# lucidrains/audiolm-pytorch

Measured on NVIDIA H100. Metric: CoarseTransformer tokens/sec fwd+bwd seq2048, higher is better.
Workload: dtype bf16

## Files before the change

audiolm_pytorch_b200/csrc/attn_fwd_wgmma.cu:

```cuda
#include "alm_common.cuh"
#include "ptx_sm90.cuh"

namespace alm {

constexpr int ATT_BM = 128;
constexpr int ATT_BN = 128;
constexpr int ATT_THREADS = 384;
template <int D>
struct AttFwdCfg {
  static constexpr int KV_STAGES = D == 128 ? 3 : 4;
  static constexpr int HALF_BYTES = 128 * SwizzledTile<D>::ROW_BYTES;
  static constexpr int TILE_BYTES = 128 * D * 2;
  static constexpr int SMEM_BYTES = TILE_BYTES * (1 + 2 * KV_STAGES) + 256;
};

struct AttnFwdParams {
  __nv_bfloat16* o;
  float* lse;
  const uint32_t* kmask;
  int kb_stride;
  const float* bias;
  long long bias_hs, bias_rs;
  long long ldo, lse_stride;
  int b, h, n_q, n_k;
  int causal;
  float scale_log2;
  int n_q_pad;
  uint32_t drop_row0;
  DropoutArgs drop;
};

__device__ __forceinline__ float att_ex2(float x) {
  float y;
  asm("ex2.approx.ftz.f32 %0, %1;" : "=f"(y) : "f"(x));
  return y;
}

__device__ __forceinline__ uint64_t attn_fwd_keep_bits(const DropoutArgs& d, uint32_t qrow, uint32_t kbase, int c_lane) {
  const uint32_t odd = qrow & 1u;
  uint64_t bits = 0;
#pragma unroll
  for (int kk = 0; kk < ATT_BN / 16; ++kk) {
    const uint32_t j0 = kbase + 16 * kk + c_lane;
    const uint4 own = dropout_draw(d, qrow, j0 + odd);
    const uint32_t ra = __shfl_xor_sync(0xffffffffu, odd ? own.x : own.y, 4);
    const uint32_t rb = __shfl_xor_sync(0xffffffffu, odd ? own.z : own.w, 4);
    const uint4 other = odd ? make_uint4(0u, ra, 0u, rb) : make_uint4(ra, 0u, rb, 0u);
#pragma unroll
    for (int c = 0; c < 2; ++c) {
      const uint4 dr = (uint32_t)c == odd ? own : other;
#pragma unroll
      for (int half = 0; half < 2; ++half)
#pragma unroll
        for (int h = 0; h < 2; ++h)
          if (dropout_pick(d, dr, qrow + 8 * h, j0 + 8 * half + c)) bits |= 1ull << (8 * kk + 4 * half + 2 * h + c);
    }
  }
  return bits;
}

template <int ATT_D, bool HAS_BIAS, bool DROPOUT>
__global__ void __launch_bounds__(ATT_THREADS, 1)
mqa_attn_fwd_kernel(const __grid_constant__ CUtensorMap tmQ, const __grid_constant__ CUtensorMap tmK,
                    const __grid_constant__ CUtensorMap tmV, const AttnFwdParams p) {
  using Tile = SwizzledTile<ATT_D>;
  using Cfg = AttFwdCfg<ATT_D>;
  constexpr int ATT_KV_STAGES = Cfg::KV_STAGES, ATT_TILE_BYTES = Cfg::TILE_BYTES, HALF = Cfg::HALF_BYTES;
  constexpr bool REG_HANDOFF = ATT_D == 128;
  extern __shared__ __align__(1024) uint8_t smem_raw[];
  uint8_t* smem = smem_raw;
  if ((smem_u32(smem) & 1023u) != 0) __trap();
  uint8_t* sQ = smem;
  uint8_t* sK = sQ + ATT_TILE_BYTES;
  uint8_t* sV = sK + ATT_KV_STAGES * ATT_TILE_BYTES;
  uint64_t* bars = reinterpret_cast<uint64_t*>(sV + ATT_KV_STAGES * ATT_TILE_BYTES);
  uint64_t* q_full = bars;
  uint64_t* kv_full = bars + 1;
  uint64_t* kv_empty = kv_full + ATT_KV_STAGES;

  const int warp = threadIdx.x >> 5;
  const int lane = threadIdx.x & 31;
  const int wg = warp >> 2;
  const int n_qblocks = (p.n_q + ATT_BM - 1) / ATT_BM;
  const int qb = n_qblocks - 1 - (int)blockIdx.x;
  const int head = blockIdx.y;
  const int batch = blockIdx.z;
  const int q0 = qb * ATT_BM;
  const int off = p.n_k - p.n_q;
  int kv_end = p.n_k;
  if (p.causal) kv_end = min(p.n_k, q0 + ATT_BM + off);
  const int n_tiles = kv_end > 0 ? (kv_end + ATT_BN - 1) / ATT_BN : 0;

  if (threadIdx.x == 0) {
    tma_prefetch_desc(&tmQ);
    tma_prefetch_desc(&tmK);
    tma_prefetch_desc(&tmV);
    mbar_init(q_full, 1);
    for (int i = 0; i < ATT_KV_STAGES; ++i) {
      mbar_init(&kv_full[i], 1);
      mbar_init(&kv_empty[i], 8);
    }
    fence_mbar_init();
  }
  __syncthreads();

  if (wg == 0) {
    if constexpr (REG_HANDOFF) setmaxnreg_dec<40>();
    if (warp == 0 && n_tiles > 0) {
      if (elect_one_sync()) {
        mbar_arrive_expect_tx(q_full, ATT_TILE_BYTES);
#pragma unroll
        for (int hf = 0; hf < Tile::HALVES; ++hf)
          tma_load_3d(sQ + hf * HALF, &tmQ, q_full, head * ATT_D + hf * Tile::HW, q0, batch);
      }
      __syncwarp();
      int stage = 0;
      uint32_t phase = 0;
      for (int j = 0; j < n_tiles; ++j) {
        mbar_wait(&kv_empty[stage], phase ^ 1u);
        if (elect_one_sync()) {
          mbar_arrive_expect_tx(&kv_full[stage], 2 * ATT_TILE_BYTES);
#pragma unroll
          for (int hf = 0; hf < Tile::HALVES; ++hf) {
            tma_load_3d(sK + stage * ATT_TILE_BYTES + hf * HALF, &tmK, &kv_full[stage], hf * Tile::HW, j * ATT_BN, batch);
            tma_load_3d(sV + stage * ATT_TILE_BYTES + hf * HALF, &tmV, &kv_full[stage], hf * Tile::HW, j * ATT_BN, batch);
          }
        }
        __syncwarp();
        if (++stage == ATT_KV_STAGES) { stage = 0; phase ^= 1u; }
      }
    }
    return;
  }

  if constexpr (REG_HANDOFF) setmaxnreg_inc<232>();
  const int cw = wg - 1;
  const int r_base = cw * 64 + (warp & 3) * 16 + (lane >> 2);
  const int c_lane = 2 * (lane & 3);
  constexpr float kLog2e = 1.4426950408889634f;
  float m_run[2] = {-INFINITY, -INFINITY}, l_run[2] = {0.f, 0.f};
  float o_acc[ATT_D / 2];
#pragma unroll
  for (int d = 0; d < ATT_D / 2; ++d) o_acc[d] = 0.f;
  int q_limit[2];
  [[maybe_unused]] const float* brow[2];
#pragma unroll
  for (int h = 0; h < 2; ++h) {
    const int qi = q0 + r_base + 8 * h;
    q_limit[h] = min(p.causal ? qi + off : p.n_k - 1, p.n_k - 1);
    if constexpr (HAS_BIAS) brow[h] = p.bias + (long long)head * p.bias_hs + (long long)min(qi, p.n_q - 1) * p.bias_rs;
  }
  const uint32_t* mrow = p.kmask ? p.kmask + (long long)batch * p.kb_stride : nullptr;
  const uint32_t q_addr = smem_u32(sQ) + cw * 64 * Tile::ROW_BYTES;
  [[maybe_unused]] const uint32_t drop_row =
      p.drop_row0 + ((uint32_t)batch * p.h + head) * (uint32_t)p.n_q_pad + q0 + r_base;

  if (n_tiles > 0) mbar_wait(q_full, 0);
  int stage = 0;
  uint32_t phase = 0;
  for (int j = 0; j < n_tiles; ++j) {
    mbar_wait(&kv_full[stage], phase);
    const uint32_t k_addr = smem_u32(sK + stage * ATT_TILE_BYTES);
    const uint32_t v_addr = smem_u32(sV + stage * ATT_TILE_BYTES);
    float s[ATT_BN / 2];
    wgmma_fence();
#pragma unroll
    for (int k = 0; k < ATT_D / 16; ++k)
      wgmma_ss<ATT_BN>(s, Tile::kmajor(q_addr, k, HALF), Tile::kmajor(k_addr, k, HALF), k > 0 ? 1u : 0u);
    wgmma_commit();
    [[maybe_unused]] uint64_t keep = 0;
    if constexpr (DROPOUT) keep = attn_fwd_keep_bits(p.drop, drop_row, j * ATT_BN, c_lane);
    wgmma_wait<0>();
    wgmma_fence_acc(s);

    const int kbase = j * ATT_BN;
    const bool tile_full = mrow == nullptr && kbase + ATT_BN <= p.n_k && (!p.causal || kbase + ATT_BN - 1 <= q0 + off);
    uint32_t valid[4] = {0xFFFFFFFFu, 0xFFFFFFFFu, 0xFFFFFFFFu, 0xFFFFFFFFu};
    if (!tile_full && mrow != nullptr) {
      const uint4 mv = __ldg(reinterpret_cast<const uint4*>(mrow + j * 4));
      valid[0] = mv.x; valid[1] = mv.y; valid[2] = mv.z; valid[3] = mv.w;
    }
    uint32_t pa[ATT_BN / 16][4];
#pragma unroll
    for (int h = 0; h < 2; ++h) {
#pragma unroll
      for (int g = 0; g < ATT_BN / 8; ++g)
#pragma unroll
        for (int c = 0; c < 2; ++c) {
          const int col = 8 * g + c_lane + c;
          float v = s[4 * g + 2 * h + c] * p.scale_log2;
          if constexpr (HAS_BIAS) {
            if (kbase + col < p.bias_rs) v = fmaf(__ldg(brow[h] + kbase + col), kLog2e, v);
          }
          if (!tile_full) {
            const bool ok = kbase + col <= q_limit[h] && ((valid[col >> 5] >> (col & 31)) & 1u);
            if (!ok) v = -INFINITY;
          }
          s[4 * g + 2 * h + c] = v;
        }
      float m_tile = -INFINITY;
#pragma unroll
      for (int g = 0; g < ATT_BN / 8; ++g) m_tile = fmaxf(m_tile, fmaxf(s[4 * g + 2 * h], s[4 * g + 2 * h + 1]));
      m_tile = fmaxf(m_tile, __shfl_xor_sync(0xffffffffu, m_tile, 1));
      m_tile = fmaxf(m_tile, __shfl_xor_sync(0xffffffffu, m_tile, 2));
      const float m_new = fmaxf(m_run[h], m_tile);
      const float m_use = (m_new == -INFINITY) ? 0.f : m_new;
      const float alpha = att_ex2(m_run[h] - m_use);
      float l_tile = 0.f;
#pragma unroll
      for (int g = 0; g < ATT_BN / 8; ++g)
#pragma unroll
        for (int c = 0; c < 2; ++c) {
          const float pv = att_ex2(s[4 * g + 2 * h + c] - m_use);
          s[4 * g + 2 * h + c] = pv;
          l_tile += pv;
        }
      l_run[h] = fmaf(l_run[h], alpha, l_tile);
      m_run[h] = m_new;
#pragma unroll
      for (int g = 0; g < ATT_D / 8; ++g) {
        o_acc[4 * g + 2 * h] *= alpha;
        o_acc[4 * g + 2 * h + 1] *= alpha;
      }
    }
    if constexpr (DROPOUT) {
#pragma unroll
      for (int e = 0; e < ATT_BN / 2; ++e) s[e] = ((keep >> e) & 1u) ? s[e] * p.drop.scale : 0.f;
    }
#pragma unroll
    for (int kk = 0; kk < ATT_BN / 16; ++kk) {
      pa[kk][0] = pack_bf16x2(s[8 * kk + 0], s[8 * kk + 1]);
      pa[kk][1] = pack_bf16x2(s[8 * kk + 2], s[8 * kk + 3]);
      pa[kk][2] = pack_bf16x2(s[8 * kk + 4], s[8 * kk + 5]);
      pa[kk][3] = pack_bf16x2(s[8 * kk + 6], s[8 * kk + 7]);
    }
    wgmma_fence_acc(o_acc);
    wgmma_fence();
#pragma unroll
    for (int kk = 0; kk < ATT_BN / 16; ++kk)
      wgmma_rs<ATT_D, 1>(o_acc, pa[kk], Tile::mnmajor(v_addr, kk, HALF), 1u);
    wgmma_commit();
    wgmma_wait<0>();
    wgmma_fence_acc(o_acc);
    if (lane == 0) mbar_arrive(&kv_empty[stage]);
    if (++stage == ATT_KV_STAGES) { stage = 0; phase ^= 1u; }
  }

#pragma unroll
  for (int h = 0; h < 2; ++h) {
    float l_tot = l_run[h];
    l_tot += __shfl_xor_sync(0xffffffffu, l_tot, 1);
    l_tot += __shfl_xor_sync(0xffffffffu, l_tot, 2);
    const int qi = q0 + r_base + 8 * h;
    if (qi < p.n_q) {
      const float inv = l_tot > 0.f ? 1.f / l_tot : 0.f;
      __nv_bfloat16* dst = p.o + ((long long)batch * p.n_q + qi) * p.ldo + head * ATT_D + c_lane;
#pragma unroll
      for (int g = 0; g < ATT_D / 8; ++g)
        *reinterpret_cast<uint32_t*>(dst + 8 * g) = pack_bf16x2(o_acc[4 * g + 2 * h] * inv, o_acc[4 * g + 2 * h + 1] * inv);
      if (p.lse != nullptr && (lane & 3) == 0) {
        const float lse = l_tot > 0.f ? (m_run[h] + log2f(l_tot)) : INFINITY;
        p.lse[((long long)batch * p.h + head) * p.lse_stride + qi] = lse;
      }
    }
  }
}

}

namespace alm {
__global__ void pack_key_mask_kernel(const uint8_t* __restrict__ mask, uint32_t* __restrict__ bits, int n_k, int words,
                                     long long total) {
  const long long i = (long long)blockIdx.x * (blockDim.x >> 5) + (threadIdx.x >> 5);
  if (i >= total) return;
  const long long b = i / words;
  const int k = (int)(i - b * words) * 32 + (threadIdx.x & 31);
  const bool on = k < n_k && mask[b * n_k + k] != 0;
  const uint32_t v = __ballot_sync(0xffffffffu, on);
  if ((threadIdx.x & 31) == 0) bits[i] = v;
}
}

extern "C" int alm_pack_key_mask(const void* key_mask, void* bits, int b, int n_k, alm_stream_t stream_) {
  using namespace alm;
  cudaStream_t stream = reinterpret_cast<cudaStream_t>(stream_);
  ALM_REQUIRE(key_mask && bits && b > 0 && n_k > 0, ALM_ERR_ARG);
  const int words = (n_k + 127) / 128 * 4;
  const long long total = (long long)b * words;
  const long long blocks = ceil_div(total, 8LL);
  ALM_REQUIRE(blocks <= INT_MAX, ALM_ERR_UNSUPPORTED);
  pack_key_mask_kernel<<<(unsigned)blocks, 256, 0, stream>>>(reinterpret_cast<const uint8_t*>(key_mask),
                                                            reinterpret_cast<uint32_t*>(bits), n_k, words, total);
  ALM_CHECK_LAUNCH();
  ALM_LAUNCHED(1);
  return ALM_OK;
}

namespace alm {
template <int D>
static int attn_fwd_launch(const void* q, int64_t ldq, const void* k, int64_t ldk, int64_t k_bstride, const void* v,
                           int64_t ldv, int64_t v_bstride, const void* key_mask, void* o, int64_t ldo, float* lse,
                           const float* bias, int b, bool drop, AttnFwdParams p, cudaStream_t stream) {
  using Tile = SwizzledTile<D>;
  constexpr int SMEM = AttFwdCfg<D>::SMEM_BYTES;
  const int h = p.h, n_q = p.n_q, n_k = p.n_k;
  static bool attr_set = false;
  if (!attr_set) {
    ALM_CUDA_OK(cudaFuncSetAttribute(mqa_attn_fwd_kernel<D, false, false>, cudaFuncAttributeMaxDynamicSharedMemorySize, SMEM));
    ALM_CUDA_OK(cudaFuncSetAttribute(mqa_attn_fwd_kernel<D, true, false>, cudaFuncAttributeMaxDynamicSharedMemorySize, SMEM));
    ALM_CUDA_OK(cudaFuncSetAttribute(mqa_attn_fwd_kernel<D, false, true>, cudaFuncAttributeMaxDynamicSharedMemorySize, SMEM));
    ALM_CUDA_OK(cudaFuncSetAttribute(mqa_attn_fwd_kernel<D, true, true>, cudaFuncAttributeMaxDynamicSharedMemorySize, SMEM));
    attr_set = true;
  }
  constexpr int kMaxGridZ = 65535;
  const int n_launch = ceil_div(b, kMaxGridZ);
  for (int b0 = 0; b0 < b; b0 += kMaxGridZ) {
    const int nb = min(b - b0, kMaxGridZ);
    CUtensorMap tmQ, tmK, tmV;
    {
      uint64_t dims[3] = {(uint64_t)h * D, (uint64_t)n_q, (uint64_t)nb};
      uint64_t strides[3] = {2, (uint64_t)ldq * 2, (uint64_t)n_q * ldq * 2};
      uint32_t box[3] = {Tile::HW, ATT_BM, 1};
      int rc = make_tensor_map(&tmQ, reinterpret_cast<const __nv_bfloat16*>(q) + (long long)b0 * n_q * ldq, 2, 3, dims,
                               strides, box, Tile::SWIZZLE);
      if (rc != ALM_OK) return rc;
    }
    {
      uint64_t dims[3] = {(uint64_t)D, (uint64_t)n_k, (uint64_t)nb};
      uint64_t strides[3] = {2, (uint64_t)ldk * 2, (uint64_t)k_bstride * 2};
      uint32_t box[3] = {Tile::HW, ATT_BN, 1};
      int rc = make_tensor_map(&tmK, reinterpret_cast<const __nv_bfloat16*>(k) + (long long)b0 * k_bstride, 2, 3, dims,
                               strides, box, Tile::SWIZZLE);
      if (rc != ALM_OK) return rc;
      strides[1] = (uint64_t)ldv * 2;
      strides[2] = (uint64_t)v_bstride * 2;
      rc = make_tensor_map(&tmV, reinterpret_cast<const __nv_bfloat16*>(v) + (long long)b0 * v_bstride, 2, 3, dims,
                           strides, box, Tile::SWIZZLE);
      if (rc != ALM_OK) return rc;
    }
    p.o = reinterpret_cast<__nv_bfloat16*>(o) + (long long)b0 * n_q * ldo;
    p.lse = lse != nullptr ? lse + (long long)b0 * h * p.lse_stride : nullptr;
    p.kmask = key_mask != nullptr ? reinterpret_cast<const uint32_t*>(key_mask) + (long long)b0 * p.kb_stride : nullptr;
    p.b = nb;
    p.drop_row0 = (uint32_t)((long long)b0 * h * p.n_q_pad);
    const dim3 grid((n_q + ATT_BM - 1) / ATT_BM, h, nb);
    if (bias != nullptr && drop)
      mqa_attn_fwd_kernel<D, true, true><<<grid, ATT_THREADS, SMEM, stream>>>(tmQ, tmK, tmV, p);
    else if (bias != nullptr)
      mqa_attn_fwd_kernel<D, true, false><<<grid, ATT_THREADS, SMEM, stream>>>(tmQ, tmK, tmV, p);
    else if (drop)
      mqa_attn_fwd_kernel<D, false, true><<<grid, ATT_THREADS, SMEM, stream>>>(tmQ, tmK, tmV, p);
    else
      mqa_attn_fwd_kernel<D, false, false><<<grid, ATT_THREADS, SMEM, stream>>>(tmQ, tmK, tmV, p);
    ALM_CHECK_LAUNCH();
  }
  ALM_LAUNCHED(n_launch);
  return ALM_OK;
}
}

extern "C" int alm_mqa_attn_fwd_dh(const void* q, int64_t ldq, const void* k, int64_t ldk, int64_t k_bstride,
                                   const void* v, int64_t ldv, int64_t v_bstride, const void* key_mask, void* o,
                                   int64_t ldo, float* lse, int64_t lse_stride, const float* bias,
                                   int64_t bias_hstride, int64_t bias_rstride, int b, int h, int n_q, int n_k,
                                   int causal, float scale, float dropout_p, uint64_t seed, uint32_t site,
                                   int dim_head, alm_stream_t stream_) {
  using namespace alm;
  cudaStream_t stream = reinterpret_cast<cudaStream_t>(stream_);
  ALM_REQUIRE(dim_head == 32 || dim_head == 64 || dim_head == 128, ALM_ERR_UNSUPPORTED);
  ALM_REQUIRE(q && k && v && o, ALM_ERR_ARG);
  ALM_REQUIRE(b > 0 && h > 0 && n_q > 0 && n_k > 0 && n_k >= n_q, ALM_ERR_ARG);
  ALM_REQUIRE(dropout_p >= 0.f && dropout_p < 1.f, ALM_ERR_ARG);
  ALM_REQUIRE((long long)b * h * ((n_q + 127) / 128 * 128) < (1ll << 32), ALM_ERR_UNSUPPORTED);
  ALM_REQUIRE(ldq % 8 == 0 && ldk % 8 == 0 && ldv % 8 == 0 && ldo % 8 == 0, ALM_ERR_ALIGN);
  ALM_REQUIRE(k_bstride % 8 == 0 && v_bstride % 8 == 0, ALM_ERR_ALIGN);
  ALM_REQUIRE((reinterpret_cast<uintptr_t>(o) & 15u) == 0, ALM_ERR_ALIGN);
  if (bias != nullptr) {
    ALM_REQUIRE(bias_rstride >= n_k && bias_rstride % 4 == 0 && bias_hstride % 4 == 0, ALM_ERR_ALIGN);
    ALM_REQUIRE((reinterpret_cast<uintptr_t>(bias) & 15u) == 0, ALM_ERR_ALIGN);
  }

  AttnFwdParams p;
  p.kb_stride = (n_k + 127) / 128 * 4;
  p.bias = bias;
  p.bias_hs = bias_hstride;
  p.bias_rs = bias_rstride;
  p.ldo = ldo;
  p.lse_stride = lse_stride;
  p.h = h; p.n_q = n_q; p.n_k = n_k;
  p.causal = causal;
  p.scale_log2 = scale * 1.4426950408889634f;
  p.n_q_pad = (n_q + 127) / 128 * 128;
  p.drop = make_dropout_args(dropout_p, seed, site);
  const bool drop = dropout_p > 0.f;
#define ALM_ATT_FWD(DD) \
  attn_fwd_launch<DD>(q, ldq, k, ldk, k_bstride, v, ldv, v_bstride, key_mask, o, ldo, lse, bias, b, drop, p, stream)
  if (dim_head == 32) return ALM_ATT_FWD(32);
  if (dim_head == 64) return ALM_ATT_FWD(64);
  return ALM_ATT_FWD(128);
#undef ALM_ATT_FWD
}

extern "C" int alm_mqa_attn_fwd(const void* q, int64_t ldq, const void* k, int64_t ldk, int64_t k_bstride,
                                const void* v, int64_t ldv, int64_t v_bstride, const void* key_mask, void* o,
                                int64_t ldo, float* lse, int64_t lse_stride, const float* bias, int64_t bias_hstride,
                                int64_t bias_rstride, int b, int h, int n_q, int n_k, int causal, float scale,
                                float dropout_p, uint64_t seed, uint32_t site, alm_stream_t stream_) {
  return alm_mqa_attn_fwd_dh(q, ldq, k, ldk, k_bstride, v, ldv, v_bstride, key_mask, o, ldo, lse, lse_stride, bias,
                             bias_hstride, bias_rstride, b, h, n_q, n_k, causal, scale, dropout_p, seed, site, 64,
                             stream_);
}
```

audiolm_pytorch_b200/csrc/ptx_sm90.cuh:

```cuda
#pragma once
#include <cuda.h>
#include <cuda_runtime.h>
#include <cuda_bf16.h>
#include <stdint.h>
#include <stdio.h>

namespace alm {

__device__ __forceinline__ uint32_t smem_u32(const void* p) {
  return static_cast<uint32_t>(__cvta_generic_to_shared(p));
}
__device__ __forceinline__ uint32_t lane_id() { return threadIdx.x & 31u; }

__device__ __forceinline__ uint64_t global_timer_ns() {
  uint64_t t;
  asm volatile("mov.u64 %0, %%globaltimer;" : "=l"(t));
  return t;
}

__device__ __forceinline__ void mbar_init(uint64_t* bar, uint32_t arrive_count) {
  asm volatile("mbarrier.init.shared::cta.b64 [%0], %1;" ::"r"(smem_u32(bar)), "r"(arrive_count) : "memory");
}
__device__ __forceinline__ void fence_mbar_init() {
  asm volatile("fence.mbarrier_init.release.cluster;" ::: "memory");
}
__device__ __forceinline__ void mbar_arrive(uint64_t* bar) {
  asm volatile("mbarrier.arrive.shared::cta.b64 _, [%0];" ::"r"(smem_u32(bar)) : "memory");
}
__device__ __forceinline__ void mbar_arrive_expect_tx(uint64_t* bar, uint32_t tx_bytes) {
  asm volatile("mbarrier.arrive.expect_tx.shared::cta.b64 _, [%0], %1;" ::"r"(smem_u32(bar)), "r"(tx_bytes)
               : "memory");
}
__device__ __forceinline__ bool mbar_try_wait(uint64_t* bar, uint32_t parity) {
  uint32_t done;
  asm volatile(
      "{\n\t"
      ".reg .pred p;\n\t"
      "mbarrier.try_wait.parity.shared::cta.b64 p, [%1], %2;\n\t"
      "selp.u32 %0, 1, 0, p;\n\t"
      "}\n"
      : "=r"(done)
      : "r"(smem_u32(bar)), "r"(parity)
      : "memory");
  return done != 0;
}
#ifndef ALM_MBAR_TIMEOUT_NS
#define ALM_MBAR_TIMEOUT_NS 4000000000ull
#endif
__device__ __forceinline__ void mbar_wait(uint64_t* bar, uint32_t parity) {
  if (mbar_try_wait(bar, parity)) return;
  uint64_t t0 = 0;
  uint32_t spins = 0;
  while (!mbar_try_wait(bar, parity)) {
    if ((++spins & 0x3FFu) == 0) {
      uint64_t now = global_timer_ns();
      if (t0 == 0) t0 = now;
      else if (now - t0 > ALM_MBAR_TIMEOUT_NS) __trap();
    }
  }
}

__device__ __forceinline__ void fence_proxy_async_smem() {
  asm volatile("fence.proxy.async.shared::cta;" ::: "memory");
}

__device__ __forceinline__ void tma_prefetch_desc(const CUtensorMap* m) {
  asm volatile("prefetch.tensormap [%0];" ::"l"(reinterpret_cast<uint64_t>(m)) : "memory");
}
__device__ __forceinline__ void tma_load_2d(void* smem_dst, const CUtensorMap* m, uint64_t* bar, int32_t c0,
                                            int32_t c1) {
  asm volatile(
      "cp.async.bulk.tensor.2d.shared::cluster.global.mbarrier::complete_tx::bytes [%0], [%1, {%3, %4}], [%2];"
      ::"r"(smem_u32(smem_dst)), "l"(reinterpret_cast<uint64_t>(m)), "r"(smem_u32(bar)), "r"(c0), "r"(c1)
      : "memory");
}
__device__ __forceinline__ void tma_load_3d(void* smem_dst, const CUtensorMap* m, uint64_t* bar, int32_t c0,
                                            int32_t c1, int32_t c2) {
  asm volatile(
      "cp.async.bulk.tensor.3d.shared::cluster.global.mbarrier::complete_tx::bytes [%0], [%1, {%3, %4, %5}], [%2];"
      ::"r"(smem_u32(smem_dst)), "l"(reinterpret_cast<uint64_t>(m)), "r"(smem_u32(bar)), "r"(c0), "r"(c1), "r"(c2)
      : "memory");
}
__device__ __forceinline__ void tma_store_3d(const CUtensorMap* m, const void* smem_src, int32_t c0, int32_t c1,
                                             int32_t c2) {
  asm volatile("cp.async.bulk.tensor.3d.global.shared::cta.bulk_group [%0, {%2, %3, %4}], [%1];"
               ::"l"(reinterpret_cast<uint64_t>(m)), "r"(smem_u32(smem_src)), "r"(c0), "r"(c1), "r"(c2)
               : "memory");
}
__device__ __forceinline__ void tma_reduce_add_3d(const CUtensorMap* m, uint32_t smem_src, int32_t c0, int32_t c1,
                                                  int32_t c2) {
  asm volatile("cp.reduce.async.bulk.tensor.3d.global.shared::cta.add.bulk_group [%0, {%2, %3, %4}], [%1];"
               ::"l"(reinterpret_cast<uint64_t>(m)), "r"(smem_src), "r"(c0), "r"(c1), "r"(c2)
               : "memory");
}
__device__ __forceinline__ void bulk_commit_group() { asm volatile("cp.async.bulk.commit_group;" ::: "memory"); }
template <int N>
__device__ __forceinline__ void bulk_wait_group_read() {
  asm volatile("cp.async.bulk.wait_group.read %0;" ::"n"(N) : "memory");
}
template <int N>
__device__ __forceinline__ void bulk_wait_group() {
  asm volatile("cp.async.bulk.wait_group %0;" ::"n"(N) : "memory");
}
__device__ __forceinline__ void st_shared_u32(uint32_t smem_addr, uint32_t v) {
  asm volatile("st.shared.u32 [%0], %1;" ::"r"(smem_addr), "r"(v) : "memory");
}
__device__ __forceinline__ void st_shared_f32x2(uint32_t smem_addr, float a, float b) {
  asm volatile("st.shared.v2.f32 [%0], {%1, %2};" ::"r"(smem_addr), "f"(a), "f"(b) : "memory");
}
__device__ __forceinline__ void named_bar_sync(uint32_t id, uint32_t nthreads) {
  asm volatile("bar.sync %0, %1;" ::"r"(id), "r"(nthreads) : "memory");
}
__device__ __forceinline__ uint64_t wgmma_desc_sw128(uint32_t smem_addr, uint32_t sbo_bytes, uint32_t lbo_bytes) {
  uint32_t lo = ((smem_addr >> 4) & 0x3FFFu) | (((lbo_bytes >> 4) & 0x3FFFu) << 16);
  uint32_t hi = ((sbo_bytes >> 4) & 0x3FFFu) | (1u << 30);
  return (static_cast<uint64_t>(hi) << 32) | lo;
}
__device__ __forceinline__ uint64_t wgmma_desc_sw64(uint32_t smem_addr, uint32_t sbo_bytes, uint32_t lbo_bytes) {
  uint32_t lo = ((smem_addr >> 4) & 0x3FFFu) | (((lbo_bytes >> 4) & 0x3FFFu) << 16);
  uint32_t hi = ((sbo_bytes >> 4) & 0x3FFFu) | (2u << 30);
  return (static_cast<uint64_t>(hi) << 32) | lo;
}
template <int W>
struct SwizzledTile {
  static constexpr int HW = W < 64 ? W : 64;
  static constexpr int HALVES = W / HW;
  static constexpr int ROW_BYTES = HW * 2;
  static constexpr int SWIZZLE = ROW_BYTES;
  static_assert(W == 32 || W == 64 || W == 128, "tile widths of the attention kernels");
  static __device__ __forceinline__ uint64_t desc(uint32_t addr, uint32_t lbo) {
    return SWIZZLE == 128 ? wgmma_desc_sw128(addr, 8 * ROW_BYTES, lbo) : wgmma_desc_sw64(addr, 8 * ROW_BYTES, lbo);
  }
  static __device__ __forceinline__ uint64_t kmajor(uint32_t addr, int k, uint32_t half_bytes) {
    return desc(addr + (k / (HW / 16)) * half_bytes + (k % (HW / 16)) * 32, 16);
  }
  static __device__ __forceinline__ uint64_t mnmajor(uint32_t addr, int kk, uint32_t half_bytes) {
    return desc(addr + kk * 16 * ROW_BYTES, half_bytes);
  }
};
__device__ __forceinline__ uint64_t wgmma_desc_nosw(uint32_t smem_addr, uint32_t sbo_bytes, uint32_t lbo_bytes) {
  uint32_t lo = ((smem_addr >> 4) & 0x3FFFu) | (((lbo_bytes >> 4) & 0x3FFFu) << 16);
  uint32_t hi = ((sbo_bytes >> 4) & 0x3FFFu);
  return (static_cast<uint64_t>(hi) << 32) | lo;
}
__device__ __forceinline__ void wgmma_fence() { asm volatile("wgmma.fence.sync.aligned;" ::: "memory"); }
__device__ __forceinline__ void wgmma_commit() { asm volatile("wgmma.commit_group.sync.aligned;" ::: "memory"); }
template <int N>
__device__ __forceinline__ void wgmma_wait() {
  asm volatile("wgmma.wait_group.sync.aligned %0;" ::"n"(N) : "memory");
}
template <int R>
__device__ __forceinline__ void wgmma_fence_acc(float (&d)[R]) {
#pragma unroll
  for (int i = 0; i < R; ++i) asm volatile("" : "+f"(d[i])::"memory");
}
template <int N>
__device__ __forceinline__ void setmaxnreg_inc() {
  asm volatile("setmaxnreg.inc.sync.aligned.u32 %0;" ::"n"(N));
}
template <int N>
__device__ __forceinline__ void setmaxnreg_dec() {
  asm volatile("setmaxnreg.dec.sync.aligned.u32 %0;" ::"n"(N));
}

template <int TA, int TB>
__device__ __forceinline__ void wgmma_ss_n32(float (&d)[16], uint64_t da, uint64_t db, uint32_t accumulate) {
  asm volatile(
      "{\n\t.reg .pred p;\n\tsetp.ne.b32 p, %18, 0;\n\t"
      "wgmma.mma_async.sync.aligned.m64n32k16.f32.bf16.bf16 {%0, %1, %2, %3, %4, %5, %6, %7, %8, %9, %10, %11, %12, %13, %14, %15}, %16, %17, p, 1, 1, %19, %20;\n\t}\n"
      : "+f"(d[0]), "+f"(d[1]), "+f"(d[2]), "+f"(d[3]), "+f"(d[4]), "+f"(d[5]), "+f"(d[6]), "+f"(d[7]), "+f"(d[8]), "+f"(d[9]), "+f"(d[10]), "+f"(d[11]), "+f"(d[12]), "+f"(d[13]), "+f"(d[14]), "+f"(d[15])
      : "l"(da), "l"(db), "r"(accumulate), "n"(TA), "n"(TB));
}

template <int TA, int TB>
__device__ __forceinline__ void wgmma_ss_n64(float (&d)[32], uint64_t da, uint64_t db, uint32_t accumulate) {
  asm volatile(
      "{\n\t.reg .pred p;\n\tsetp.ne.b32 p, %34, 0;\n\t"
      "wgmma.mma_async.sync.aligned.m64n64k16.f32.bf16.bf16 {%0, %1, %2, %3, %4, %5, %6, %7, %8, %9, %10, %11, %12, %13, %14, %15, %16, %17, %18, %19, %20, %21, %22, %23, %24, %25, %26, %27, %28, %29, %30, %31}, %32, %33, p, 1, 1, %35, %36;\n\t}\n"
      : "+f"(d[0]), "+f"(d[1]), "+f"(d[2]), "+f"(d[3]), "+f"(d[4]), "+f"(d[5]), "+f"(d[6]), "+f"(d[7]), "+f"(d[8]), "+f"(d[9]), "+f"(d[10]), "+f"(d[11]), "+f"(d[12]), "+f"(d[13]), "+f"(d[14]), "+f"(d[15]), "+f"(d[16]), "+f"(d[17]), "+f"(d[18]), "+f"(d[19]), "+f"(d[20]), "+f"(d[21]), "+f"(d[22]), "+f"(d[23]), "+f"(d[24]), "+f"(d[25]), "+f"(d[26]), "+f"(d[27]), "+f"(d[28]), "+f"(d[29]), "+f"(d[30]), "+f"(d[31])
      : "l"(da), "l"(db), "r"(accumulate), "n"(TA), "n"(TB));
}
template <int TB>
__device__ __forceinline__ void wgmma_rs_n64(float (&d)[32], const uint32_t (&a)[4], uint64_t db, uint32_t accumulate) {
  asm volatile(
      "{\n\t.reg .pred p;\n\tsetp.ne.b32 p, %37, 0;\n\t"
      "wgmma.mma_async.sync.aligned.m64n64k16.f32.bf16.bf16 {%0, %1, %2, %3, %4, %5, %6, %7, %8, %9, %10, %11, %12, %13, %14, %15, %16, %17, %18, %19, %20, %21, %22, %23, %24, %25, %26, %27, %28, %29, %30, %31}, {%32, %33, %34, %35}, %36, p, 1, 1, %38;\n\t}\n"
      : "+f"(d[0]), "+f"(d[1]), "+f"(d[2]), "+f"(d[3]), "+f"(d[4]), "+f"(d[5]), "+f"(d[6]), "+f"(d[7]), "+f"(d[8]), "+f"(d[9]), "+f"(d[10]), "+f"(d[11]), "+f"(d[12]), "+f"(d[13]), "+f"(d[14]), "+f"(d[15]), "+f"(d[16]), "+f"(d[17]), "+f"(d[18]), "+f"(d[19]), "+f"(d[20]), "+f"(d[21]), "+f"(d[22]), "+f"(d[23]), "+f"(d[24]), "+f"(d[25]), "+f"(d[26]), "+f"(d[27]), "+f"(d[28]), "+f"(d[29]), "+f"(d[30]), "+f"(d[31])
      : "r"(a[0]), "r"(a[1]), "r"(a[2]), "r"(a[3]), "l"(db), "r"(accumulate), "n"(TB));
}

template <int TA, int TB>
__device__ __forceinline__ void wgmma_ss_n128(float (&d)[64], uint64_t da, uint64_t db, uint32_t accumulate) {
  asm volatile(
      "{\n\t.reg .pred p;\n\tsetp.ne.b32 p, %66, 0;\n\t"
      "wgmma.mma_async.sync.aligned.m64n128k16.f32.bf16.bf16 {%0, %1, %2, %3, %4, %5, %6, %7, %8, %9, %10, %11, %12, %13, %14, %15, %16, %17, %18, %19, %20, %21, %22, %23, %24, %25, %26, %27, %28, %29, %30, %31, %32, %33, %34, %35, %36, %37, %38, %39, %40, %41, %42, %43, %44, %45, %46, %47, %48, %49, %50, %51, %52, %53, %54, %55, %56, %57, %58, %59, %60, %61, %62, %63}, %64, %65, p, 1, 1, %67, %68;\n\t}\n"
      : "+f"(d[0]), "+f"(d[1]), "+f"(d[2]), "+f"(d[3]), "+f"(d[4]), "+f"(d[5]), "+f"(d[6]), "+f"(d[7]), "+f"(d[8]), "+f"(d[9]), "+f"(d[10]), "+f"(d[11]), "+f"(d[12]), "+f"(d[13]), "+f"(d[14]), "+f"(d[15]), "+f"(d[16]), "+f"(d[17]), "+f"(d[18]), "+f"(d[19]), "+f"(d[20]), "+f"(d[21]), "+f"(d[22]), "+f"(d[23]), "+f"(d[24]), "+f"(d[25]), "+f"(d[26]), "+f"(d[27]), "+f"(d[28]), "+f"(d[29]), "+f"(d[30]), "+f"(d[31]), "+f"(d[32]), "+f"(d[33]), "+f"(d[34]), "+f"(d[35]), "+f"(d[36]), "+f"(d[37]), "+f"(d[38]), "+f"(d[39]), "+f"(d[40]), "+f"(d[41]), "+f"(d[42]), "+f"(d[43]), "+f"(d[44]), "+f"(d[45]), "+f"(d[46]), "+f"(d[47]), "+f"(d[48]), "+f"(d[49]), "+f"(d[50]), "+f"(d[51]), "+f"(d[52]), "+f"(d[53]), "+f"(d[54]), "+f"(d[55]), "+f"(d[56]), "+f"(d[57]), "+f"(d[58]), "+f"(d[59]), "+f"(d[60]), "+f"(d[61]), "+f"(d[62]), "+f"(d[63])
      : "l"(da), "l"(db), "r"(accumulate), "n"(TA), "n"(TB));
}

template <int TA, int TB>
__device__ __forceinline__ void wgmma_ss_n256(float (&d)[128], uint64_t da, uint64_t db, uint32_t accumulate) {
  asm volatile(
      "{\n\t.reg .pred p;\n\tsetp.ne.b32 p, %130, 0;\n\t"
      "wgmma.mma_async.sync.aligned.m64n256k16.f32.bf16.bf16 {%0, %1, %2, %3, %4, %5, %6, %7, %8, %9, %10, %11, %12, %13, %14, %15, %16, %17, %18, %19, %20, %21, %22, %23, %24, %25, %26, %27, %28, %29, %30, %31, %32, %33, %34, %35, %36, %37, %38, %39, %40, %41, %42, %43, %44, %45, %46, %47, %48, %49, %50, %51, %52, %53, %54, %55, %56, %57, %58, %59, %60, %61, %62, %63, %64, %65, %66, %67, %68, %69, %70, %71, %72, %73, %74, %75, %76, %77, %78, %79, %80, %81, %82, %83, %84, %85, %86, %87, %88, %89, %90, %91, %92, %93, %94, %95, %96, %97, %98, %99, %100, %101, %102, %103, %104, %105, %106, %107, %108, %109, %110, %111, %112, %113, %114, %115, %116, %117, %118, %119, %120, %121, %122, %123, %124, %125, %126, %127}, %128, %129, p, 1, 1, %131, %132;\n\t}\n"
      : "+f"(d[0]), "+f"(d[1]), "+f"(d[2]), "+f"(d[3]), "+f"(d[4]), "+f"(d[5]), "+f"(d[6]), "+f"(d[7]), "+f"(d[8]), "+f"(d[9]), "+f"(d[10]), "+f"(d[11]), "+f"(d[12]), "+f"(d[13]), "+f"(d[14]), "+f"(d[15]), "+f"(d[16]), "+f"(d[17]), "+f"(d[18]), "+f"(d[19]), "+f"(d[20]), "+f"(d[21]), "+f"(d[22]), "+f"(d[23]), "+f"(d[24]), "+f"(d[25]), "+f"(d[26]), "+f"(d[27]), "+f"(d[28]), "+f"(d[29]), "+f"(d[30]), "+f"(d[31]), "+f"(d[32]), "+f"(d[33]), "+f"(d[34]), "+f"(d[35]), "+f"(d[36]), "+f"(d[37]), "+f"(d[38]), "+f"(d[39]), "+f"(d[40]), "+f"(d[41]), "+f"(d[42]), "+f"(d[43]), "+f"(d[44]), "+f"(d[45]), "+f"(d[46]), "+f"(d[47]), "+f"(d[48]), "+f"(d[49]), "+f"(d[50]), "+f"(d[51]), "+f"(d[52]), "+f"(d[53]), "+f"(d[54]), "+f"(d[55]), "+f"(d[56]), "+f"(d[57]), "+f"(d[58]), "+f"(d[59]), "+f"(d[60]), "+f"(d[61]), "+f"(d[62]), "+f"(d[63]), "+f"(d[64]), "+f"(d[65]), "+f"(d[66]), "+f"(d[67]), "+f"(d[68]), "+f"(d[69]), "+f"(d[70]), "+f"(d[71]), "+f"(d[72]), "+f"(d[73]), "+f"(d[74]), "+f"(d[75]), "+f"(d[76]), "+f"(d[77]), "+f"(d[78]), "+f"(d[79]), "+f"(d[80]), "+f"(d[81]), "+f"(d[82]), "+f"(d[83]), "+f"(d[84]), "+f"(d[85]), "+f"(d[86]), "+f"(d[87]), "+f"(d[88]), "+f"(d[89]), "+f"(d[90]), "+f"(d[91]), "+f"(d[92]), "+f"(d[93]), "+f"(d[94]), "+f"(d[95]), "+f"(d[96]), "+f"(d[97]), "+f"(d[98]), "+f"(d[99]), "+f"(d[100]), "+f"(d[101]), "+f"(d[102]), "+f"(d[103]), "+f"(d[104]), "+f"(d[105]), "+f"(d[106]), "+f"(d[107]), "+f"(d[108]), "+f"(d[109]), "+f"(d[110]), "+f"(d[111]), "+f"(d[112]), "+f"(d[113]), "+f"(d[114]), "+f"(d[115]), "+f"(d[116]), "+f"(d[117]), "+f"(d[118]), "+f"(d[119]), "+f"(d[120]), "+f"(d[121]), "+f"(d[122]), "+f"(d[123]), "+f"(d[124]), "+f"(d[125]), "+f"(d[126]), "+f"(d[127])
      : "l"(da), "l"(db), "r"(accumulate), "n"(TA), "n"(TB));
}

template <int TB>
__device__ __forceinline__ void wgmma_rs_n32(float (&d)[16], const uint32_t (&a)[4], uint64_t db, uint32_t accumulate) {
  asm volatile(
      "{\n\t.reg .pred p;\n\tsetp.ne.b32 p, %21, 0;\n\t"
      "wgmma.mma_async.sync.aligned.m64n32k16.f32.bf16.bf16 {%0, %1, %2, %3, %4, %5, %6, %7, %8, %9, %10, %11, %12, %13, %14, %15}, {%16, %17, %18, %19}, %20, p, 1, 1, %22;\n\t}\n"
      : "+f"(d[0]), "+f"(d[1]), "+f"(d[2]), "+f"(d[3]), "+f"(d[4]), "+f"(d[5]), "+f"(d[6]), "+f"(d[7]), "+f"(d[8]), "+f"(d[9]), "+f"(d[10]), "+f"(d[11]), "+f"(d[12]), "+f"(d[13]), "+f"(d[14]), "+f"(d[15])
      : "r"(a[0]), "r"(a[1]), "r"(a[2]), "r"(a[3]), "l"(db), "r"(accumulate), "n"(TB));
}
template <int TB>
__device__ __forceinline__ void wgmma_rs_n128(float (&d)[64], const uint32_t (&a)[4], uint64_t db, uint32_t accumulate) {
  asm volatile(
      "{\n\t.reg .pred p;\n\tsetp.ne.b32 p, %69, 0;\n\t"
      "wgmma.mma_async.sync.aligned.m64n128k16.f32.bf16.bf16 {%0, %1, %2, %3, %4, %5, %6, %7, %8, %9, %10, %11, %12, %13, %14, %15, %16, %17, %18, %19, %20, %21, %22, %23, %24, %25, %26, %27, %28, %29, %30, %31, %32, %33, %34, %35, %36, %37, %38, %39, %40, %41, %42, %43, %44, %45, %46, %47, %48, %49, %50, %51, %52, %53, %54, %55, %56, %57, %58, %59, %60, %61, %62, %63}, {%64, %65, %66, %67}, %68, p, 1, 1, %70;\n\t}\n"
      : "+f"(d[0]), "+f"(d[1]), "+f"(d[2]), "+f"(d[3]), "+f"(d[4]), "+f"(d[5]), "+f"(d[6]), "+f"(d[7]), "+f"(d[8]), "+f"(d[9]), "+f"(d[10]), "+f"(d[11]), "+f"(d[12]), "+f"(d[13]), "+f"(d[14]), "+f"(d[15]), "+f"(d[16]), "+f"(d[17]), "+f"(d[18]), "+f"(d[19]), "+f"(d[20]), "+f"(d[21]), "+f"(d[22]), "+f"(d[23]), "+f"(d[24]), "+f"(d[25]), "+f"(d[26]), "+f"(d[27]), "+f"(d[28]), "+f"(d[29]), "+f"(d[30]), "+f"(d[31]), "+f"(d[32]), "+f"(d[33]), "+f"(d[34]), "+f"(d[35]), "+f"(d[36]), "+f"(d[37]), "+f"(d[38]), "+f"(d[39]), "+f"(d[40]), "+f"(d[41]), "+f"(d[42]), "+f"(d[43]), "+f"(d[44]), "+f"(d[45]), "+f"(d[46]), "+f"(d[47]), "+f"(d[48]), "+f"(d[49]), "+f"(d[50]), "+f"(d[51]), "+f"(d[52]), "+f"(d[53]), "+f"(d[54]), "+f"(d[55]), "+f"(d[56]), "+f"(d[57]), "+f"(d[58]), "+f"(d[59]), "+f"(d[60]), "+f"(d[61]), "+f"(d[62]), "+f"(d[63])
      : "r"(a[0]), "r"(a[1]), "r"(a[2]), "r"(a[3]), "l"(db), "r"(accumulate), "n"(TB));
}

template <int TB>
__device__ __forceinline__ void wgmma_rs_n256(float (&d)[128], const uint32_t (&a)[4], uint64_t db, uint32_t accumulate) {
  asm volatile(
      "{\n\t.reg .pred p;\n\tsetp.ne.b32 p, %133, 0;\n\t"
      "wgmma.mma_async.sync.aligned.m64n256k16.f32.bf16.bf16 {%0, %1, %2, %3, %4, %5, %6, %7, %8, %9, %10, %11, %12, %13, %14, %15, %16, %17, %18, %19, %20, %21, %22, %23, %24, %25, %26, %27, %28, %29, %30, %31, %32, %33, %34, %35, %36, %37, %38, %39, %40, %41, %42, %43, %44, %45, %46, %47, %48, %49, %50, %51, %52, %53, %54, %55, %56, %57, %58, %59, %60, %61, %62, %63, %64, %65, %66, %67, %68, %69, %70, %71, %72, %73, %74, %75, %76, %77, %78, %79, %80, %81, %82, %83, %84, %85, %86, %87, %88, %89, %90, %91, %92, %93, %94, %95, %96, %97, %98, %99, %100, %101, %102, %103, %104, %105, %106, %107, %108, %109, %110, %111, %112, %113, %114, %115, %116, %117, %118, %119, %120, %121, %122, %123, %124, %125, %126, %127}, {%128, %129, %130, %131}, %132, p, 1, 1, %134;\n\t}\n"
      : "+f"(d[0]), "+f"(d[1]), "+f"(d[2]), "+f"(d[3]), "+f"(d[4]), "+f"(d[5]), "+f"(d[6]), "+f"(d[7]), "+f"(d[8]), "+f"(d[9]), "+f"(d[10]), "+f"(d[11]), "+f"(d[12]), "+f"(d[13]), "+f"(d[14]), "+f"(d[15]), "+f"(d[16]), "+f"(d[17]), "+f"(d[18]), "+f"(d[19]), "+f"(d[20]), "+f"(d[21]), "+f"(d[22]), "+f"(d[23]), "+f"(d[24]), "+f"(d[25]), "+f"(d[26]), "+f"(d[27]), "+f"(d[28]), "+f"(d[29]), "+f"(d[30]), "+f"(d[31]), "+f"(d[32]), "+f"(d[33]), "+f"(d[34]), "+f"(d[35]), "+f"(d[36]), "+f"(d[37]), "+f"(d[38]), "+f"(d[39]), "+f"(d[40]), "+f"(d[41]), "+f"(d[42]), "+f"(d[43]), "+f"(d[44]), "+f"(d[45]), "+f"(d[46]), "+f"(d[47]), "+f"(d[48]), "+f"(d[49]), "+f"(d[50]), "+f"(d[51]), "+f"(d[52]), "+f"(d[53]), "+f"(d[54]), "+f"(d[55]), "+f"(d[56]), "+f"(d[57]), "+f"(d[58]), "+f"(d[59]), "+f"(d[60]), "+f"(d[61]), "+f"(d[62]), "+f"(d[63]), "+f"(d[64]), "+f"(d[65]), "+f"(d[66]), "+f"(d[67]), "+f"(d[68]), "+f"(d[69]), "+f"(d[70]), "+f"(d[71]), "+f"(d[72]), "+f"(d[73]), "+f"(d[74]), "+f"(d[75]), "+f"(d[76]), "+f"(d[77]), "+f"(d[78]), "+f"(d[79]), "+f"(d[80]), "+f"(d[81]), "+f"(d[82]), "+f"(d[83]), "+f"(d[84]), "+f"(d[85]), "+f"(d[86]), "+f"(d[87]), "+f"(d[88]), "+f"(d[89]), "+f"(d[90]), "+f"(d[91]), "+f"(d[92]), "+f"(d[93]), "+f"(d[94]), "+f"(d[95]), "+f"(d[96]), "+f"(d[97]), "+f"(d[98]), "+f"(d[99]), "+f"(d[100]), "+f"(d[101]), "+f"(d[102]), "+f"(d[103]), "+f"(d[104]), "+f"(d[105]), "+f"(d[106]), "+f"(d[107]), "+f"(d[108]), "+f"(d[109]), "+f"(d[110]), "+f"(d[111]), "+f"(d[112]), "+f"(d[113]), "+f"(d[114]), "+f"(d[115]), "+f"(d[116]), "+f"(d[117]), "+f"(d[118]), "+f"(d[119]), "+f"(d[120]), "+f"(d[121]), "+f"(d[122]), "+f"(d[123]), "+f"(d[124]), "+f"(d[125]), "+f"(d[126]), "+f"(d[127])
      : "r"(a[0]), "r"(a[1]), "r"(a[2]), "r"(a[3]), "l"(db), "r"(accumulate), "n"(TB));
}

template <int N, int TA = 0, int TB = 0>
__device__ __forceinline__ void wgmma_ss(float (&d)[N / 2], uint64_t da, uint64_t db, uint32_t accumulate) {
  if constexpr (N == 32) wgmma_ss_n32<TA, TB>(d, da, db, accumulate);
  else if constexpr (N == 64) wgmma_ss_n64<TA, TB>(d, da, db, accumulate);
  else if constexpr (N == 128) wgmma_ss_n128<TA, TB>(d, da, db, accumulate);
  else wgmma_ss_n256<TA, TB>(d, da, db, accumulate);
}
template <int N, int TB = 0>
__device__ __forceinline__ void wgmma_rs(float (&d)[N / 2], const uint32_t (&a)[4], uint64_t db, uint32_t accumulate) {
  static_assert(N == 32 || N == 64 || N == 128 || N == 256, "the register-A form is instantiated for N = 32 ... 256");
  if constexpr (N == 32) wgmma_rs_n32<TB>(d, a, db, accumulate);
  else if constexpr (N == 64) wgmma_rs_n64<TB>(d, a, db, accumulate);
  else if constexpr (N == 128) wgmma_rs_n128<TB>(d, a, db, accumulate);
  else wgmma_rs_n256<TB>(d, a, db, accumulate);
}

__device__ __forceinline__ uint32_t pack_bf16x2(float lo, float hi) {
  __nv_bfloat162 v = __floats2bfloat162_rn(lo, hi);
  return *reinterpret_cast<uint32_t*>(&v);
}

__device__ __forceinline__ bool elect_one_sync() {
  uint32_t pred;
  asm volatile(
      "{\n\t"
      ".reg .pred p;\n\t"
      "elect.sync _|p, 0xffffffff;\n\t"
      "selp.u32 %0, 1, 0, p;\n\t"
      "}\n"
      : "=r"(pred));
  return pred != 0;
}
__device__ __forceinline__ void bulk_copy_g2s(void* smem_dst, const void* gsrc, uint32_t bytes, uint64_t* bar) {
  asm volatile("cp.async.bulk.shared::cluster.global.mbarrier::complete_tx::bytes [%0], [%1], %2, [%3];" ::"r"(
                   smem_u32(smem_dst)),
               "l"(reinterpret_cast<uint64_t>(gsrc)), "r"(bytes), "r"(smem_u32(bar))
               : "memory");
}
__device__ __forceinline__ void split_bf16(float x, __nv_bfloat16& hi, __nv_bfloat16& lo) {
  hi = __float2bfloat16_rn(x);
  lo = __float2bfloat16_rn(x - __bfloat162float(hi));
}

__device__ __forceinline__ void cp_async_16(void* smem_dst, const void* gsrc, uint32_t src_bytes = 16) {
  asm volatile("cp.async.cg.shared.global [%0], [%1], 16, %2;" ::"r"(smem_u32(smem_dst)),
               "l"(reinterpret_cast<uint64_t>(gsrc)), "r"(src_bytes)
               : "memory");
}
__device__ __forceinline__ void prefetch_l2(const void* gaddr) {
  asm volatile("prefetch.global.L2 [%0];" ::"l"(reinterpret_cast<uint64_t>(gaddr)));
}
__device__ __forceinline__ void cp_async_commit() { asm volatile("cp.async.commit_group;" ::: "memory"); }
template <int N>
__device__ __forceinline__ void cp_async_wait() {
  asm volatile("cp.async.wait_group %0;" ::"n"(N) : "memory");
}
__device__ __forceinline__ void split_bf16x2(float a, float b, uint32_t& hi, uint32_t& lo) {
  asm("cvt.rn.bf16x2.f32 %0, %1, %2;" : "=r"(hi) : "f"(b), "f"(a));
  const float ra = a - __uint_as_float(hi << 16);
  const float rb = b - __uint_as_float(hi & 0xFFFF0000u);
  asm("cvt.rn.bf16x2.f32 %0, %1, %2;" : "=r"(lo) : "f"(rb), "f"(ra));
}

}
```

Baseline: 744,600.

## Pipeline QK and PV wgmma with ping-pong warpgroup scheduling in attention forward

For head dims 32 and 64 (without bias or dropout at 64), the consumer loop now issues the next tile's QK^T wgmma together with the previous tile's PV wgmma. Two consumer warpgroups take turns issuing via named barriers (ping-pong), so softmax of one overlaps tensor-core work of the other. Masking is precomputed into per-lane bitmasks, bias loads are vectorized, and the register handoff now applies at all head dims. This adds register pressure from keeping two tiles live, plus extra barrier synchronization.

```diff
diff --git a/audiolm_pytorch_b200/csrc/attn_fwd_wgmma.cu b/audiolm_pytorch_b200/csrc/attn_fwd_wgmma.cu
--- a/audiolm_pytorch_b200/csrc/attn_fwd_wgmma.cu
+++ b/audiolm_pytorch_b200/csrc/attn_fwd_wgmma.cu
@@ -6,6 +6,7 @@
 constexpr int ATT_BM = 128;
 constexpr int ATT_BN = 128;
 constexpr int ATT_THREADS = 384;
+constexpr uint32_t ATT_TURN_BAR = 1;
 template <int D>
 struct AttFwdCfg {
   static constexpr int KV_STAGES = D == 128 ? 3 : 4;
@@ -66,7 +67,7 @@
   using Tile = SwizzledTile<ATT_D>;
   using Cfg = AttFwdCfg<ATT_D>;
   constexpr int ATT_KV_STAGES = Cfg::KV_STAGES, ATT_TILE_BYTES = Cfg::TILE_BYTES, HALF = Cfg::HALF_BYTES;
-  constexpr bool REG_HANDOFF = ATT_D == 128;
+  constexpr bool PIPELINED = ATT_D == 32 || (ATT_D == 64 && !HAS_BIAS && !DROPOUT);
   extern __shared__ __align__(1024) uint8_t smem_raw[];
   uint8_t* smem = smem_raw;
   if ((smem_u32(smem) & 1023u) != 0) __trap();
@@ -105,7 +106,7 @@
   __syncthreads();
 
   if (wg == 0) {
-    if constexpr (REG_HANDOFF) setmaxnreg_dec<40>();
+    setmaxnreg_dec<40>();
     if (warp == 0 && n_tiles > 0) {
       if (elect_one_sync()) {
         mbar_arrive_expect_tx(q_full, ATT_TILE_BYTES);
@@ -133,7 +134,7 @@
     return;
   }
 
-  if constexpr (REG_HANDOFF) setmaxnreg_inc<232>();
+  setmaxnreg_inc<232>();
   const int cw = wg - 1;
   const int r_base = cw * 64 + (warp & 3) * 16 + (lane >> 2);
   const int c_lane = 2 * (lane & 3);
@@ -155,49 +156,76 @@
   [[maybe_unused]] const uint32_t drop_row =
       p.drop_row0 + ((uint32_t)batch * p.h + head) * (uint32_t)p.n_q_pad + q0 + r_base;
 
-  if (n_tiles > 0) mbar_wait(q_full, 0);
-  int stage = 0;
-  uint32_t phase = 0;
-  for (int j = 0; j < n_tiles; ++j) {
-    mbar_wait(&kv_full[stage], phase);
-    const uint32_t k_addr = smem_u32(sK + stage * ATT_TILE_BYTES);
-    const uint32_t v_addr = smem_u32(sV + stage * ATT_TILE_BYTES);
-    float s[ATT_BN / 2];
+  uint32_t pa[ATT_BN / 16][4];
+  auto issue_qk = [&](float (&s)[ATT_BN / 2], int st) {
+    const uint32_t k_addr = smem_u32(sK + st * ATT_TILE_BYTES);
     wgmma_fence();
 #pragma unroll
     for (int k = 0; k < ATT_D / 16; ++k)
       wgmma_ss<ATT_BN>(s, Tile::kmajor(q_addr, k, HALF), Tile::kmajor(k_addr, k, HALF), k > 0 ? 1u : 0u);
     wgmma_commit();
-    [[maybe_unused]] uint64_t keep = 0;
-    if constexpr (DROPOUT) keep = attn_fwd_keep_bits(p.drop, drop_row, j * ATT_BN, c_lane);
-    wgmma_wait<0>();
-    wgmma_fence_acc(s);
-
+  };
+  auto issue_pv = [&](int st) {
+    const uint32_t v_addr = smem_u32(sV + st * ATT_TILE_BYTES);
+    wgmma_fence_acc(o_acc);
+    wgmma_fence();
+#pragma unroll
+    for (int kk = 0; kk < ATT_BN / 16; ++kk)
+      wgmma_rs<ATT_D, 1>(o_acc, pa[kk], Tile::mnmajor(v_addr, kk, HALF), 1u);
+    wgmma_commit();
+  };
+  auto key_bits = [&](int j) {
+    uint4 mv = make_uint4(0xFFFFFFFFu, 0xFFFFFFFFu, 0xFFFFFFFFu, 0xFFFFFFFFu);
+    if (mrow != nullptr) mv = __ldg(reinterpret_cast<const uint4*>(mrow + j * 4));
+    return mv;
+  };
+  auto softmax = [&](float (&s)[ATT_BN / 2], int j, const uint4 mv, float (&alpha)[2]) {
     const int kbase = j * ATT_BN;
     const bool tile_full = mrow == nullptr && kbase + ATT_BN <= p.n_k && (!p.causal || kbase + ATT_BN - 1 <= q0 + off);
-    uint32_t valid[4] = {0xFFFFFFFFu, 0xFFFFFFFFu, 0xFFFFFFFFu, 0xFFFFFFFFu};
-    if (!tile_full && mrow != nullptr) {
-      const uint4 mv = __ldg(reinterpret_cast<const uint4*>(mrow + j * 4));
-      valid[0] = mv.x; valid[1] = mv.y; valid[2] = mv.z; valid[3] = mv.w;
-    }
-    uint32_t pa[ATT_BN / 16][4];
+    const uint32_t valid[4] = {mv.x, mv.y, mv.z, mv.w};
+    uint32_t vis[2] = {0xFFFFFFFFu, 0xFFFFFFFFu};
+    if (ATT_D != 128 && !tile_full) {
+      uint32_t keys = 0;
+#pragma unroll
+      for (int g = 0; g < ATT_BN / 8; ++g) keys |= ((valid[g >> 2] >> (8 * (g & 3) + c_lane)) & 3u) << (2 * g);
+#pragma unroll
+      for (int h = 0; h < 2; ++h) {
+        const int last = q_limit[h] - kbase - c_lane;
+        const int n0 = last < 0 ? 0 : min(last / 8 + 1, ATT_BN / 8);
+        const int n1 = last < 1 ? 0 : min((last - 1) / 8 + 1, ATT_BN / 8);
+        const int n_vis = n0 + n1;
+        vis[h] = keys & (n_vis >= 32 ? 0xFFFFFFFFu : (1u << n_vis) - 1u);
+      }
+    }
 #pragma unroll
     for (int h = 0; h < 2; ++h) {
-#pragma unroll
-      for (int g = 0; g < ATT_BN / 8; ++g)
+      [[maybe_unused]] const float* bt = nullptr;
+      [[maybe_unused]] int blim = 0;
+      if constexpr (HAS_BIAS) {
+        bt = brow[h] + kbase + c_lane;
+        blim = (int)min(p.bias_rs - kbase - c_lane, (long long)ATT_BN);
+      }
+#pragma unroll
+      for (int g = 0; g < ATT_BN / 8; ++g) {
+        [[maybe_unused]] float2 bb = make_float2(0.f, 0.f);
+        if constexpr (HAS_BIAS) {
+          if (8 * g < blim) bb = __ldg(reinterpret_cast<const float2*>(bt + 8 * g));
+        }
 #pragma unroll
         for (int c = 0; c < 2; ++c) {
-          const int col = 8 * g + c_lane + c;
           float v = s[4 * g + 2 * h + c] * p.scale_log2;
           if constexpr (HAS_BIAS) {
-            if (kbase + col < p.bias_rs) v = fmaf(__ldg(brow[h] + kbase + col), kLog2e, v);
+            if (8 * g < blim) v = fmaf(c == 0 ? bb.x : bb.y, kLog2e, v);
           }
-          if (!tile_full) {
-            const bool ok = kbase + col <= q_limit[h] && ((valid[col >> 5] >> (col & 31)) & 1u);
-            if (!ok) v = -INFINITY;
+          if constexpr (ATT_D != 128) {
+            if (!((vis[h] >> (2 * g + c)) & 1u)) v = -INFINITY;
+          } else if (!tile_full) {
+            const int col = 8 * g + c_lane + c;
+            if (!(kbase + col <= q_limit[h] && ((valid[col >> 5] >> (col & 31)) & 1u))) v = -INFINITY;
           }
           s[4 * g + 2 * h + c] = v;
         }
+      }
       float m_tile = -INFINITY;
 #pragma unroll
       for (int g = 0; g < ATT_BN / 8; ++g) m_tile = fmaxf(m_tile, fmaxf(s[4 * g + 2 * h], s[4 * g + 2 * h + 1]));
@@ -205,7 +233,7 @@
       m_tile = fmaxf(m_tile, __shfl_xor_sync(0xffffffffu, m_tile, 2));
       const float m_new = fmaxf(m_run[h], m_tile);
       const float m_use = (m_new == -INFINITY) ? 0.f : m_new;
-      const float alpha = att_ex2(m_run[h] - m_use);
+      alpha[h] = att_ex2(m_run[h] - m_use);
       float l_tile = 0.f;
 #pragma unroll
       for (int g = 0; g < ATT_BN / 8; ++g)
@@ -215,14 +243,18 @@
           s[4 * g + 2 * h + c] = pv;
           l_tile += pv;
         }
-      l_run[h] = fmaf(l_run[h], alpha, l_tile);
+      l_run[h] = fmaf(l_run[h], alpha[h], l_tile);
       m_run[h] = m_new;
+    }
+  };
+  auto rescale_and_pack = [&](float (&s)[ATT_BN / 2], const float (&alpha)[2], uint64_t keep) {
+#pragma unroll
+    for (int h = 0; h < 2; ++h)
 #pragma unroll
       for (int g = 0; g < ATT_D / 8; ++g) {
-        o_acc[4 * g + 2 * h] *= alpha;
-        o_acc[4 * g + 2 * h + 1] *= alpha;
-      }
-    }
+        o_acc[4 * g + 2 * h] *= alpha[h];
+        o_acc[4 * g + 2 * h + 1] *= alpha[h];
+      }
     if constexpr (DROPOUT) {
 #pragma unroll
       for (int e = 0; e < ATT_BN / 2; ++e) s[e] = ((keep >> e) & 1u) ? s[e] * p.drop.scale : 0.f;
@@ -234,16 +266,71 @@
       pa[kk][2] = pack_bf16x2(s[8 * kk + 4], s[8 * kk + 5]);
       pa[kk][3] = pack_bf16x2(s[8 * kk + 6], s[8 * kk + 7]);
     }
-    wgmma_fence_acc(o_acc);
-    wgmma_fence();
-#pragma unroll
-    for (int kk = 0; kk < ATT_BN / 16; ++kk)
-      wgmma_rs<ATT_D, 1>(o_acc, pa[kk], Tile::mnmajor(v_addr, kk, HALF), 1u);
-    wgmma_commit();
+  };
+
+  mbar_wait(q_full, 0);
+  int stage = 0;
+  uint32_t phase = 0;
+  if constexpr (PIPELINED) {
+    const uint32_t my_turn = ATT_TURN_BAR + cw, other_turn = ATT_TURN_BAR + (cw ^ 1);
+    if (cw == 1) named_bar_arrive(other_turn, 256);
+    mbar_wait(&kv_full[0], 0);
+    {
+      float s[ATT_BN / 2], alpha[2];
+      named_bar_sync(my_turn, 256);
+      issue_qk(s, 0);
+      named_bar_arrive(other_turn, 256);
+      [[maybe_unused]] uint64_t keep = 0;
+      if constexpr (DROPOUT) keep = attn_fwd_keep_bits(p.drop, drop_row, 0, c_lane);
+      const uint4 mv = key_bits(0);
+      wgmma_wait<0>();
+      wgmma_fence_acc(s);
+      softmax(s, 0, mv, alpha);
+      rescale_and_pack(s, alpha, keep);
+    }
+    for (int j = 1; j < n_tiles; ++j) {
+      const int prev = stage;
+      if (++stage == ATT_KV_STAGES) { stage = 0; phase ^= 1u; }
+      mbar_wait(&kv_full[stage], phase);
+      float s[ATT_BN / 2], alpha[2];
+      named_bar_sync(my_turn, 256);
+      issue_qk(s, stage);
+      issue_pv(prev);
+      named_bar_arrive(other_turn, 256);
+      [[maybe_unused]] uint64_t keep = 0;
+      if constexpr (DROPOUT) keep = attn_fwd_keep_bits(p.drop, drop_row, j * ATT_BN, c_lane);
+      const uint4 mv = key_bits(j);
+      wgmma_wait<1>();
+      wgmma_fence_acc(s);
+      softmax(s, j, mv, alpha);
+      wgmma_wait<0>();
+      wgmma_fence_acc(o_acc);
+      if (lane == 0) mbar_arrive(&kv_empty[prev]);
+      rescale_and_pack(s, alpha, keep);
+    }
+    named_bar_sync(my_turn, 256);
+    issue_pv(stage);
+    if (cw == 0) named_bar_arrive(other_turn, 256);
     wgmma_wait<0>();
     wgmma_fence_acc(o_acc);
-    if (lane == 0) mbar_arrive(&kv_empty[stage]);
-    if (++stage == ATT_KV_STAGES) { stage = 0; phase ^= 1u; }
+  } else {
+    for (int j = 0; j < n_tiles; ++j) {
+      mbar_wait(&kv_full[stage], phase);
+      float s[ATT_BN / 2], alpha[2];
+      issue_qk(s, stage);
+      [[maybe_unused]] uint64_t keep = 0;
+      if constexpr (DROPOUT) keep = attn_fwd_keep_bits(p.drop, drop_row, j * ATT_BN, c_lane);
+      const uint4 mv = key_bits(j);
+      wgmma_wait<0>();
+      wgmma_fence_acc(s);
+      softmax(s, j, mv, alpha);
+      rescale_and_pack(s, alpha, keep);
+      issue_pv(stage);
+      wgmma_wait<0>();
+      wgmma_fence_acc(o_acc);
+      if (lane == 0) mbar_arrive(&kv_empty[stage]);
+      if (++stage == ATT_KV_STAGES) { stage = 0; phase ^= 1u; }
+    }
   }
 
 #pragma unroll
diff --git a/audiolm_pytorch_b200/csrc/ptx_sm90.cuh b/audiolm_pytorch_b200/csrc/ptx_sm90.cuh
--- a/audiolm_pytorch_b200/csrc/ptx_sm90.cuh
+++ b/audiolm_pytorch_b200/csrc/ptx_sm90.cuh
@@ -110,6 +110,9 @@
 }
 __device__ __forceinline__ void named_bar_sync(uint32_t id, uint32_t nthreads) {
   asm volatile("bar.sync %0, %1;" ::"r"(id), "r"(nthreads) : "memory");
+}
+__device__ __forceinline__ void named_bar_arrive(uint32_t id, uint32_t nthreads) {
+  asm volatile("bar.arrive %0, %1;" ::"r"(id), "r"(nthreads) : "memory");
 }
 __device__ __forceinline__ uint64_t wgmma_desc_sw128(uint32_t smem_addr, uint32_t sbo_bytes, uint32_t lbo_bytes) {
   uint32_t lo = ((smem_addr >> 4) & 0x3FFFu) | (((lbo_bytes >> 4) & 0x3FFFu) << 16);
```

After: 753,900 (median of 6 runs). Within noise of the previous version (+1.3%).
